# xmh1011/go-lsm

Hardware: AMD Instinct MI355X
Metric: GiB/s of device-resident .sst data-block bytes decoded to KV records (higher is better)
Workload: dtype u8; 1 GPU; decode 100000 x 4 KiB KV blocks per GPU (33 x 16 B key / 100 B value); grammar=KV (kv/kv.go:46-115), output=DESC (16 B record descriptors), blocks_per_gpu=100000, records_per_gpu=3300000, parsed_bytes_per_gpu=409200000, parallelism=dp1 (blocks round-robin, no collective)

## Files before the change

go-lsm_amd/csrc/decode.hip:

```cpp
#include <stdlib.h>
#include <string.h>

#include "common.h"

namespace lsm {
namespace {

constexpr uint32_t kChunk = 1024;
constexpr uint32_t kRingChunks = 8;
constexpr int kBlockLoadAux = 2;
constexpr uint32_t kBigLaunch = 400000;
template <uint32_t NCH, bool ARENA, bool BIG = false>
struct RingPolicy {
    static constexpr int load_aux = ((ARENA || BIG) && NCH == 8) ? 0 : kBlockLoadAux;
    static constexpr bool nt_desc = NCH == 8;
};
constexpr uint32_t kFitPad = 4096;
constexpr uint32_t kFitMin = 3072;

template <uint32_t NCH, bool ARENA>
__device__ __forceinline__ void store_desc(u32x4 *p, const u32x4 &d) {
    if (RingPolicy<NCH, ARENA>::nt_desc)
        __builtin_nontemporal_store(d, p);
    else
// ... 203 lines not shown
    constexpr uint32_t U = 1;
#pragma unroll 1
    for (uint32_t w0 = 0; w0 < nd; w0 += U * kWave) {
        uint32_t W[U], sb[U], kk[U], rr[U];
        int qv[U];
#pragma unroll
        for (uint32_t u = 0; u < U; u++) {
            const int q = (int)(4 * (w0 + u * kWave + lane)) - (int)lead;
            const uint32_t qc = q < 0 ? 0u : (uint32_t)q;
            const uint32_t r = rec(qc), o = qc - mul24(r, L);
            qv[u] = q;
            rr[u] = r;
            kk[u] = L - o;
            sb[u] = src0 + mul24(r, S) + o;
            W[u] = rb.word(sb[u] >> 2);
        }
        bool unal = false, cross = false;
#pragma unroll
        for (uint32_t u = 0; u < U; u++) {
            unal |= (sb[u] & 3) != 0;
            cross |= kk[u] < 4;
        }
        if (__ballot(unal)) {
#pragma unroll
            for (uint32_t u = 0; u < U; u++) W[u] = funnel(W[u], rb.word((sb[u] >> 2) + 1), sb[u]);
        }
        if (L < 4) {
#pragma unroll
            for (uint32_t u = 0; u < U; u++) {
                const uint32_t qc = qv[u] < 0 ? 0u : (uint32_t)qv[u];
                uint32_t x = 0;
                for (uint32_t t = 0; t < 4; t++) {
                    const uint32_t qq = qc + t;
                    if (qq < T) {
                        const uint32_t r = rec(qq);
                        x |= rb.u8(src0 + mul24(r, S) + (qq - mul24(r, L))) << (8 * t);
                    }
                }
                W[u] = x;
            }
        } else if (__ballot(cross)) {
#pragma unroll
            for (uint32_t u = 0; u < U; u++) {
                const uint32_t B = rb.u32(src0 + mul24(rr[u] + 1, S)), k = kk[u];
                W[u] = k < 4 ? (W[u] & ((1u << (8 * k)) - 1)) | (B << (8 * k)) : W[u];
            }
        }
#pragma unroll
        for (uint32_t u = 0; u < U; u++) {
            const uint32_t w = w0 + u * kWave + lane;
            const int q = qv[u];
            if (q >= 0 && (uint32_t)q + 4 <= T) {
                __builtin_nontemporal_store(W[u], &a0[w]);
            } else if (w < nd) {
                const uint32_t sh = q < 0 ? (uint32_t)(-q) : 0u;
                uint8_t *b = reinterpret_cast<uint8_t *>(a0 + w);
                for (uint32_t t = sh; t < 4 && (uint32_t)(q + (int)t) < T; t++)
                    b[t] = (uint8_t)(W[u] >> (8 * (t - sh)));
            }
        }
    }
}

template <uint32_t NCH, bool LIN>
__device__ __forceinline__ uint32_t arena_emit_batch(const RingBytes<NCH, LIN> &rb, uint32_t *tab,
                                                     uint8_t *out, uint32_t cnt, uint32_t src,
                                                     uint32_t len, uint64_t *out_off,
                                                     uint64_t cur) {
    const uint32_t lane = lane_id();
    const uint32_t l = lane < cnt ? len : 0u;
    uint32_t T;
    const uint32_t start = wave_excl_scan(l, &T);
    if (out_off && lane < cnt) out_off[lane] = cur + start;
    if (T == 0) return 0;
    uint32_t *tstart = tab, *tsrc = tab + 65;
    if (lane < cnt) {
        tstart[lane] = start;
        tsrc[lane] = src;
    }
    if (lane == 0) tstart[cnt] = T;
    __builtin_amdgcn_fence(__ATOMIC_RELEASE, "wavefront");
    __builtin_amdgcn_wave_barrier();
    __builtin_amdgcn_fence(__ATOMIC_ACQUIRE, "wavefront");
    const uint32_t lead = (uint32_t)((uintptr_t)out & 15);
    uint8_t *a0 = out - lead;
    const uint32_t nch = (lead + T + 15) >> 4;
#pragma unroll 1
    for (uint32_t c = lane; c < nch; c += kWave) {
        const int q0 = (int)(16 * c) - (int)lead;
        const uint32_t qf = q0 < 0 ? 0u : (uint32_t)q0;
        uint32_t lo = 0, hi = cnt;
        while (hi - lo > 1) {
            const uint32_t mid = (lo + hi) >> 1;
            if (tstart[mid] <= qf) lo = mid;
            else hi = mid;
        }
        uint32_t r = lo, rs0 = tstart[r], rs1 = tstart[r + 1], rsrc = tsrc[r];
        auto in_ring = [&]() { return rsrc >= rb.res_lo && rsrc + (rs1 - rs0) <= rb.res_hi; };
        auto seek = [&](uint32_t q) {
            while (rs1 <= q) {
                r++;
                rs0 = rs1;
                rs1 = tstart[r + 1];
                rsrc = tsrc[r];
            }
        };
        auto byte_at = [&](uint32_t q) -> uint32_t {
            seek(q);
            const uint32_t sb = rsrc + (q - rs0);
            return in_ring() ? rb.u8(sb) : rb.g8(sb);
        };
        u32x4 v{0, 0, 0, 0};
        if (q0 >= 0 && q0 + 16 <= (int)T && (uint32_t)q0 + 16 <= rs1) {
            const uint32_t sb = rsrc + ((uint32_t)q0 - rs0);
            if (in_ring())
                v = rb.u128(sb);
            else
                v = u32x4{rb.g32(sb), rb.g32(sb + 4), rb.g32(sb + 8), rb.g32(sb + 12)};
        } else {
#pragma unroll 1
            for (int t = 0; t < 16; t++) {
                const int q = q0 + t;
                if (q >= 0 && q < (int)T) {
                    const uint32_t b = byte_at((uint32_t)q) << (8 * (t & 3));
                    set_dword(v, (uint32_t)t >> 2, (t < 4 ? v.x : t < 8 ? v.y : t < 12 ? v.z : v.w) | b);
                }
            }
        }
        store_chunk(a0 + 16 * c, v, -q0, (int)T - q0);
    }
    __builtin_amdgcn_fence(__ATOMIC_RELEASE, "wavefront");
    __builtin_amdgcn_wave_barrier();
    __builtin_amdgcn_fence(__ATOMIC_ACQUIRE, "wavefront");
    return T;
}

typedef __attribute__((address_space(3))) uint32_t lds_u32_t;

template <uint32_t NCH, bool LIN>
__device__ __forceinline__ uint32_t arena_emit_batch_call(lds_u32_t *ring, rsrc_t rs, uint32_t res_lo,
                                                       uint32_t res_hi, lds_u32_t *tab,
                                                       uint8_t *out, uint32_t cnt, uint32_t src,
                                                       uint32_t len, uint64_t *out_off,
                                                       uint64_t cur) {
    RingBytes<NCH, LIN> rb{(const uint32_t *)ring, rs, res_lo, res_hi};
    return arena_emit_batch(rb, (uint32_t *)tab, out, cnt, src, len, out_off, cur);
}

struct ArenaCur {
    uint64_t k, v;
};

struct ChaseResume {
    uint32_t pos = 0, nr = 0, kprev = 0xFFFFFFFFu;
};
template <int G, uint32_t NCH, bool LIN, bool ARENA = false, bool BIG = false, bool PRE = false>
__device__ void decode_range_v2(const DecodeArgs &a, uint32_t *ring, uint64_t off, uint32_t n,
                                uint64_t base, uint32_t ncap, uint32_t &nr_out, int32_t &st_out,
                                uint32_t stop, uint32_t &pos_out, ArenaCur ac = {},
                                uint32_t *tab = nullptr, bool lin_rt = LIN,
                                const ChaseResume rs0 = {}) {
    static_assert(!PRE || (LIN && !ARENA), "a pre-landed ring is a DESC block that fits it");
    const bool lin = ARENA ? lin_rt : LIN;
    const uint32_t lane = lane_id();
    BlockReaderT<NCH, RingPolicy<NCH, ARENA, BIG>::load_aux> rd;
    rd.init(ring, a.in, off, n);
    RingBytes<NCH, LIN> rb{ring, rd.rsrc, 0, 0};

    auto word = [&](uint32_t w) -> uint32_t { return rb.word(w); };
    auto fld = [&](uint32_t p) -> uint32_t {
        return uni(rb.u32(rd.h + p));
    };
    auto lds_u32 = [&](uint32_t p) -> uint32_t {
        return rb.u32(rd.h + p);
    };

    uint32_t s_pos = 0, s_k = 0, s_v = 0, s_xlo = 0, s_xhi = 0, ns = 0, s_first = 0;
    uint32_t pos = rs0.pos, nr = rs0.nr, kprev = rs0.kprev, miss = 0, skip = 0;
    uint32_t pend = 0, pend_pos = 0, pend_k = 0, pend_v = 0;
    auto emit_run_arena = [&](uint32_t p0, uint32_t K, uint32_t V, uint32_t S, uint32_t cnt,
                              uint64_t slot0) {
#pragma unroll 1
        for (uint32_t f = G == LSM_GRAMMAR_V ? 1u : 0u; f < (G == LSM_GRAMMAR_IDX ? 1u : 2u);
             f++) {
            uint8_t *ar = f ? a.val_arena : a.key_arena;
            if (!ar) continue;
            uint64_t *ao = f ? a.val_arena_off : a.key_arena_off;
            const uint64_t cur = f ? ac.v : ac.k;
            const uint32_t L = f ? V : K;
            arena_emit_run(rb, ar + cur, rd.h + p0 + (f == 0 ? 4u : G == LSM_GRAMMAR_KV ? 8 + K : 4u),
                           S, L, cnt);
            if (ao)
                for (uint32_t i = lane; i < cnt; i += kWave) ao[slot0 + i] = cur + (uint64_t)i * L;
            if (f) ac.v += (uint64_t)cnt * L;
            else ac.k += (uint64_t)cnt * L;
        }
    };
    auto flush = [&]() {
        if (ns) {
            if (lane < ns) {
                const uint64_t ro = off + s_pos;
                u32x4 d;
                d.x = (uint32_t)ro;
                d.y = (uint32_t)(ro >> 32);
                d.z = s_k;
                d.w = s_v;
                store_desc<NCH, ARENA>(&a.desc[base + s_first + lane], d);
                if (G == LSM_GRAMMAR_IDX && a.idx_value)
                    a.idx_value[base + s_first + lane] = (int64_t)((uint64_t)s_xhi << 32 | s_xlo);
            }
            if (ARENA && ns > pend) {
                lds_u32_t *lring = (lds_u32_t *)ring, *ltab = (lds_u32_t *)tab;
#pragma unroll 1
                for (uint32_t f = G == LSM_GRAMMAR_V ? 1u : 0u;
                     f < (G == LSM_GRAMMAR_IDX ? 1u : 2u); f++) {
                    uint8_t *ar = f ? a.val_arena : a.key_arena;
                    if (!ar) continue;
                    uint64_t *ao = f ? a.val_arena_off : a.key_arena_off;
                    const uint64_t cur = f ? ac.v : ac.k;
                    const uint32_t src =
                        rd.h + s_pos + (f == 0 ? 4u : G == LSM_GRAMMAR_KV ? 8 + s_k : 4u);
                    const uint32_t t = arena_emit_batch_call<NCH, LIN>(
                        lring, rb.rs, rb.res_lo, rb.res_hi, ltab, ar + cur, ns - pend, src,
                        f ? s_v : s_k, ao ? ao + base + s_first : nullptr, cur);
                    if (f) ac.v += t;
                    else ac.k += t;
                }
            }
            ns = 0;
        }
    };
    uint32_t lim = PRE ? n : 0;
    auto need = [&](uint32_t p, uint32_t len) {
        if (PRE || (uint64_t)p + len <= lim) return;
        if (ARENA && !lin) {
            flush();
            if (pend) {
                emit_run_arena(pend_pos, pend_k, pend_v, 0, 1, base + nr - 1);
                pend = 0;
            }
        }
        rd.ensure(rd.h + p, lin ? rd.total : len);
        lim = rd.landed >= rd.nchunks ? n : rd.landed * kChunk - rd.h;
        if (ARENA) {
            rb.res_lo = (rd.hi_c > NCH ? rd.hi_c - NCH : 0u) * kChunk;
            rb.res_hi = rd.landed * kChunk;
        }
    };

    int32_t status = LSM_OK;
    for (;;) {
        const uint32_t rem = n - pos;
        if (rem == 0 || pos >= stop) break;
        if (rem < 4) {
            status = G == LSM_GRAMMAR_IDX ? LSM_ST_IDX_OVERRUN : LSM_ST_TRUNC_LEN_PREFIX;
            break;
        }
        need(pos, rem < kChunk ? rem : kChunk);
        uint32_t K = 0, V, S;
        uint64_t x = 0;
        if (G == LSM_GRAMMAR_V) {
            V = fld(pos);
            if (rem - 4 < V) { status = LSM_ST_TRUNC_VAL; break; }
            S = 4 + V;
        } else if (G == LSM_GRAMMAR_KV) {
            const bool sv = kprev <= kChunk - 8;
            K = fld(pos);
            const uint32_t vg = sv ? fld(pos + 4 + kprev) : 0u;
            if (K > kKeyCap) { status = LSM_ST_KEY_TOO_LONG; break; }
            if (rem - 4 < K) { status = LSM_ST_TRUNC_KEY; break; }
            const uint32_t vp = pos + 4 + K;
            const uint32_t rem2 = n - vp;
            if (rem2 < 4) { status = LSM_ST_TRUNC_VLEN; break; }
            if (sv && K == kprev) {
                V = vg;
            } else {
                need(vp, rem2 < kChunk ? rem2 : kChunk);
                V = fld(vp);
            }
            if (V > kValCap) { status = LSM_ST_VAL_TOO_LONG; break; }
            if (rem2 - 4 < V) { status = LSM_ST_TRUNC_VAL; break; }
            kprev = K;
            S = 8 + K + V;
        } else {
            K = fld(pos);
            if ((uint64_t)rem < 12ull + K) { status = LSM_ST_IDX_OVERRUN; break; }
            const uint32_t vp = pos + 4 + K;
            need(vp, 8);
            x = (uint64_t)fld(vp + 4) << 32 | fld(vp);
            V = 8;
            S = 12 + K;
        }
        if (nr >= ncap) { status = LSM_ST_CAPACITY; break; }
        if (ns == 0) s_first = nr;
        {
            const bool me = lane == ns;
            s_pos = me ? pos : s_pos;
            s_k = me ? K : s_k;
            s_v = me ? V : s_v;
            if (G == LSM_GRAMMAR_IDX) {
                s_xlo = me ? (uint32_t)x : s_xlo;
                s_xhi = me ? (uint32_t)(x >> 32) : s_xhi;
            }
        }
        if (++ns == kWave) flush();
        nr++;
        pos += S;

        if (skip) {
            skip--;
            if (G == LSM_GRAMMAR_KV && kprev <= kChunk - 8) {
                uint32_t vpos = to_vgpr(pos), kp = to_vgpr(kprev);
                while (nr < ncap) {
                    const uint32_t sb = rd.h + vpos, sv = sb + 4 + kp;
                    const uint32_t k = funnel(word(sb >> 2), word((sb >> 2) + 1), sb);
                    uint32_t v = funnel(word(sv >> 2), word((sv >> 2) + 1), sv);
                    if (!__ballot(k == kp) && __ballot(k <= kChunk - 8)) {
                        const uint32_t sw = sb + 4 + k;
                        v = funnel(word(sw >> 2), word((sw >> 2) + 1), sw);
// ... 94 lines not shown
        }
        if (ARENA && pend) {
            emit_run_arena(pend_pos, pend_k, pend_v, 0, 1, base + nr - 1);
            pend = 0;
        }
    }
    flush();
    nr_out = nr;
    st_out = status;
    pos_out = pos;
}

template <int G, uint32_t NCH, bool LIN, bool ARENA, bool BIG = false>
__device__ void decode_block_v2(const DecodeArgs &a, uint32_t b, uint32_t *ring, uint32_t *tab,
                                uint64_t off, uint32_t n, bool lin_rt = LIN) {
    uint64_t base, cap;
    record_slots<G>(a, b, off, n, base, cap);
    uint32_t nr, end;
    int32_t st;
    ArenaCur ac{};
    if (ARENA) {
        ac.k = a.arena_base ? uni64(a.arena_base[b]) : off;
        ac.v = ac.k;
    }
    decode_range_v2<G, NCH, LIN, ARENA, BIG>(a, ring, off, n, uni64(base),
                                        uni(cap < 0xFFFFFFFFull ? (uint32_t)cap : 0xFFFFFFFFu), nr,
                                        st, n, end, ac, tab, lin_rt);
    if (lane_id() == 0) {
        a.nrec[b] = nr;
        a.status[b] = st;
    }
}


template <int G, uint32_t NCH, bool BIG>
__device__ __forceinline__ void decode_block_lin(const DecodeArgs &a, uint32_t b, uint32_t *ring,
                                                 uint64_t off, uint32_t n) {
    static_assert(NCH * kChunk <= kKeyCap && NCH * kChunk <= kValCap, "caps hold for a block that fits");
    constexpr int AUX = RingPolicy<NCH, false, BIG>::load_aux;
    constexpr uint32_t R = MinRecord<G>::R;
    const uint32_t lane = lane_id();
    const uint32_t h = (uint32_t)off & 15;
    const uint32_t total = (h + n + 15) & ~15u;
    const uint32_t nchunks = (total + kChunk - 1) / kChunk;
    const rsrc_t rsrc = make_rsrc(a.in + (off - h), total);
    const uint32_t voff = lane * 16;
#pragma unroll
    for (uint32_t c = 0; c < NCH; c++)
        if (c < nchunks)
            __builtin_amdgcn_raw_ptr_buffer_load_lds(
                rsrc, (__attribute__((address_space(3))) void *)&ring[c * (kChunk / 4)], 16,
                voff + c * kChunk, 0, 0, AUX);
    uint64_t base64, cap64;
    record_slots<G>(a, b, off, n, base64, cap64);
    const uint64_t base = uni64(base64);
    const uint32_t ncap = uni(cap64 < 0xFFFFFFFFull ? (uint32_t)cap64 : 0xFFFFFFFFu);
    __asm__ __volatile__("s_waitcnt vmcnt(0)" ::: "memory");
    const RingBytes<NCH, true> rb{ring, rsrc, 0, 0};
    uint32_t pos = 0, nr = 0, K = 0, V = 8;
    if (n >= R) {
        bool ok0;
        if (G == LSM_GRAMMAR_V) {
            V = uni(rb.u32(h));
            ok0 = V <= n - 4;
        } else if (G == LSM_GRAMMAR_KV) {
            K = uni(rb.u32(h));
            ok0 = K <= n - 8;
            if (ok0) {
                V = uni(rb.u32(h + 4 + K));
                ok0 = V <= n - 8 - K;
            }
        } else {
            K = uni(rb.u32(h));
            ok0 = K <= n - 12;
        }
        if (ok0) {
            const uint32_t S = G == LSM_GRAMMAR_V ? 4 + V : G == LSM_GRAMMAR_KV ? 8 + K + V : 12 + K;
            const uint32_t p = lane * S;
            bool ok = p + S <= n && lane < ncap;
            uint64_t xx = 0;
            if (ok) {
                if (G == LSM_GRAMMAR_V) {
                    ok = rb.u32(h + p) == V;
                } else if (G == LSM_GRAMMAR_KV) {
                    ok = (int)(rb.u32(h + p) == K) & (int)(rb.u32(h + p + 4 + K) == V);
                } else {
                    ok = rb.u32(h + p) == K;
                    xx = (uint64_t)rb.u32(h + p + 8 + K) << 32 | rb.u32(h + p + 4 + K);
                }
            }
            const uint64_t m = __ballot(ok);
            const uint32_t j = m == ~0ull ? 64u : (uint32_t)__builtin_ctzll(~m);
            if (lane < j) {
                const uint64_t ro = off + p;
                u32x4 d;
                d.x = (uint32_t)ro;
                d.y = (uint32_t)(ro >> 32);
                d.z = K;
                d.w = V;
                store_desc<NCH, false>(&a.desc[base + lane], d);
                if (G == LSM_GRAMMAR_IDX && a.idx_value) a.idx_value[base + lane] = (int64_t)xx;
            }
            nr = j;
            pos = j * S;
        }
    }
    int32_t st = LSM_OK;
    if (pos != n) {
        uint32_t end;
        decode_range_v2<G, NCH, true, false, BIG, true>(
            a, ring, off, n, base, ncap, nr, st, n, end, {}, nullptr, true,
            ChaseResume{pos, nr, G == LSM_GRAMMAR_KV && nr ? K : 0xFFFFFFFFu});
    }
    if (lane == 0) {
        a.nrec[b] = nr;
        a.status[b] = st;
    }
}

template <int G, uint32_t NCH>
__device__ void decode_range_any(const DecodeArgs &a, uint32_t *ring, uint64_t off, uint32_t n,
                                 uint64_t base, uint32_t ncap, uint32_t &nr, int32_t &st,
                                 uint32_t stop = 0xFFFFFFFFu, uint32_t *end = nullptr) {
    uint32_t e;
    if (((off & 15) + (uint64_t)n + 15) / 16 * 16 <= NCH * kChunk)
        decode_range_v2<G, NCH, true>(a, ring, off, n, base, ncap, nr, st, stop, e);
    else
        decode_range_v2<G, NCH, false>(a, ring, off, n, base, ncap, nr, st, stop, e);
    if (end) *end = e;
}

template <int G, uint32_t NCH, bool ARENA, bool BIG = false, bool PAD = false>
__global__ __launch_bounds__(64) void decode_v2_kernel(DecodeArgs a) {
    static_assert(!PAD || (!ARENA && NCH == kRingChunks), "the pad is the 8 KiB DESC ring's");
    __shared__ __attribute__((aligned(16)))
    uint32_t ring[NCH * kChunk / 4 + 4 + (PAD ? kFitPad / 4 : 0)];
    __shared__ uint32_t tab[ARENA ? 129 : 1];
    const uint32_t b = a.order ? uni(a.order[blockIdx.x])
                               : NCH >= 16 ? xcd_linear(blockIdx.x, a.nblk) : blockIdx.x;
    const uint64_t off = uni64(a.blk_off[b]);
    const uint32_t n = uni(a.blk_len[b]);
    const bool lin = ((off & 15) + (uint64_t)n + 15) / 16 * 16 <= NCH * kChunk;
    if (ARENA) {
        decode_block_v2<G, NCH, false, true>(a, b, ring, tab, off, n, lin);
    } else if (lin && !BIG) {
        decode_block_lin<G, NCH, BIG>(a, b, ring, off, n);
    } else if (lin) {
        decode_block_v2<G, NCH, true, false, BIG>(a, b, ring, tab, off, n);
    } else {
        decode_block_v2<G, NCH, false, false, BIG>(a, b, ring, tab, off, n);
    }
}


constexpr uint32_t kScanThreads = 256;
constexpr uint32_t kScanPer = 2;
constexpr uint32_t kScanTile = kScanThreads * kScanPer;

__device__ __forceinline__ uint64_t plan_value(int mode, uint32_t len) {
    switch (mode) {
    case 0: return len / 4;
    case 1: return len / 8;
    case 2: return len / 12;
    default: return len;
    }
}

__device__ uint64_t block_excl_scan(uint64_t v, uint64_t *total) {
    __shared__ uint64_t wsum[kScanThreads / kWave];
    uint64_t wt;
    uint64_t x = wave_excl_scan64(v, &wt);
    uint32_t w = threadIdx.x / kWave;
    if (lane_id() == 0) wsum[w] = wt;
    __syncthreads();
    uint64_t pre = 0, tot = 0;
    for (uint32_t i = 0; i < kScanThreads / kWave; i++) {
        if (i < w) pre += wsum[i];
        tot += wsum[i];
    }
    __syncthreads();
    *total = tot;
    return x + pre;
}

__global__ __launch_bounds__(kScanThreads) void plan_tile_sums(int mode, const uint32_t *len,
                                                               uint32_t n, uint64_t *partial) {
    uint64_t s = 0;
    uint64_t i0 = (uint64_t)blockIdx.x * kScanTile + threadIdx.x * kScanPer;
    for (uint32_t j = 0; j < kScanPer; j++)
        if (i0 + j < n) s += plan_value(mode, len[i0 + j]);
    uint64_t tot;
    block_excl_scan(s, &tot);
    if (threadIdx.x == 0) partial[blockIdx.x] = tot;
}

constexpr uint32_t kPartThreads = 1024;

__global__ __launch_bounds__(kPartThreads) void plan_scan_partials(uint64_t *partial,
                                                                   uint32_t ntiles, uint64_t *out,
                                                                   uint32_t n) {
    __shared__ uint64_t wsum[kPartThreads / kWave];
    const uint32_t per = (ntiles + kPartThreads - 1) / kPartThreads, b = threadIdx.x * per;
    const uint32_t e = b + per < ntiles ? b + per : ntiles;
    uint64_t s = 0;
    for (uint32_t i0 = b; i0 < e; i0 += 8) {
        uint64_t v[8];
#pragma unroll
        for (uint32_t k = 0; k < 8; k++) v[k] = i0 + k < e ? partial[i0 + k] : 0;
#pragma unroll
        for (uint32_t k = 0; k < 8; k++) s += v[k];
    }
    uint64_t wt;
    const uint64_t wx = wave_excl_scan64(s, &wt);
    const uint32_t w = threadIdx.x / kWave;
    if (lane_id() == 0) wsum[w] = wt;
    __syncthreads();
    uint64_t pre = wx, tot = 0;
    for (uint32_t i = 0; i < kPartThreads / kWave; i++) {
        pre += i < w ? wsum[i] : 0;
        tot += wsum[i];
    }
    for (uint32_t i0 = b; i0 < e; i0 += 8) {
        uint64_t v[8];
#pragma unroll
        for (uint32_t k = 0; k < 8; k++) v[k] = i0 + k < e ? partial[i0 + k] : 0;
#pragma unroll
        for (uint32_t k = 0; k < 8; k++) {
            if (i0 + k < e) partial[i0 + k] = pre;
            pre += v[k];
        }
    }
    if (threadIdx.x == 0) out[n] = tot;
}

__global__ __launch_bounds__(kScanThreads) void plan_tile_apply(int mode, const uint32_t *len,
                                                                uint32_t n,
                                                                const uint64_t *partial,
                                                                uint64_t *out) {
    uint64_t vals[kScanPer];
    uint64_t s = 0;
    uint64_t i0 = (uint64_t)blockIdx.x * kScanTile + threadIdx.x * kScanPer;
    for (uint32_t j = 0; j < kScanPer; j++) {
        vals[j] = (i0 + j < n) ? plan_value(mode, len[i0 + j]) : 0;
        s += vals[j];
    }
    uint64_t tot;
    uint64_t pre = block_excl_scan(s, &tot) + partial[blockIdx.x];
    for (uint32_t j = 0; j < kScanPer; j++) {
        if (i0 + j < n) out[i0 + j] = pre;
        pre += vals[j];
    }
}

int plan_scan(int mode, const uint32_t *d_len, uint32_t n, uint64_t *d_out, void *ws,
              size_t ws_bytes, hipStream_t s) {
    uint32_t ntiles = (n + kScanTile - 1) / kScanTile;
    if (ntiles == 0) ntiles = 1;
    if (ws_bytes < (size_t)ntiles * 8 || (!ws && n)) return LSM_ESPACE;
    uint64_t *partial = static_cast<uint64_t *>(ws);
    if (n == 0) {
        LSM_HIP_CHECK(hipMemsetAsync(d_out, 0, 8, s));
        return 0;
    }
    hipLaunchKernelGGL(plan_tile_sums, dim3(ntiles), dim3(kScanThreads), 0, s, mode, d_len, n,
                       partial);
    hipLaunchKernelGGL(plan_scan_partials, dim3(1), dim3(kPartThreads), 0, s, partial, ntiles,
                       d_out, n);
    hipLaunchKernelGGL(plan_tile_apply, dim3(ntiles), dim3(kScanThreads), 0, s, mode, d_len, n,
                       partial, d_out);
    LSM_HIP_CHECK(hipGetLastError());
    return 0;
}

template <int G, bool ARENA, uint32_t NCH = kRingChunks>
int launch_decode(const DecodeArgs &a, hipStream_t s, bool fit = false) {
    static_assert(NCH >= 2, "a record header may straddle two ring chunks");
    constexpr bool kCanPad = !ARENA && NCH == kRingChunks && G != LSM_GRAMMAR_IDX;
    const bool big = !ARENA && NCH == kRingChunks && a.nblk > kBigLaunch && !a.order;
    if (kCanPad && fit && !big)
        hipLaunchKernelGGL((decode_v2_kernel<G, NCH, false, false, kCanPad>), dim3(a.nblk), dim3(kWave), 0, s, a);
    else if (big)
        hipLaunchKernelGGL((decode_v2_kernel<G, NCH, false, true>), dim3(a.nblk), dim3(kWave), 0, s, a);
    else
        hipLaunchKernelGGL((decode_v2_kernel<G, NCH, ARENA>), dim3(a.nblk), dim3(kWave), 0, s, a);
    LSM_HIP_CHECK(hipGetLastError());
    return 0;
}

constexpr uint32_t kSchedSub = 2;
constexpr uint32_t kSchedClasses = (33 - kSchedSub) << kSchedSub;
constexpr uint32_t kSchedThreads = 1024;
constexpr uint32_t kSchedPer = 16;
constexpr uint32_t kSchedTile = kSchedThreads * kSchedPer;
static_assert(kSchedClasses <= kSchedThreads, "one thread per class");

__device__ __forceinline__ uint32_t size_class(uint32_t n) {
    if (n < (1u << kSchedSub)) return n;
    const uint32_t l = 31 - __clz(n);
    return ((l - kSchedSub + 1) << kSchedSub) | ((n >> (l - kSchedSub)) & ((1u << kSchedSub) - 1));
}

constexpr uint32_t kSchedLaneWords = kSchedClasses * kWave;

__device__ __forceinline__ void sched_count(const uint32_t *len, uint32_t nblk, uint32_t t0,
                                            uint32_t (*h2)[kWave], uint32_t n[kSchedPer]) {
    for (uint32_t i = threadIdx.x; i < kSchedLaneWords; i += kSchedThreads) (&h2[0][0])[i] = 0;
// ... 940 lines not shown
}
size_t scan_workspace_bytes(uint32_t n) {
    const size_t ntiles = (n + kScanTile - 1) / kScanTile;
    return (ntiles ? ntiles : 1) * 8;
}
}

extern "C" uint64_t lsm_max_records(int grammar, uint64_t len) {
    switch (grammar) {
    case LSM_GRAMMAR_V: return len / 4;
    case LSM_GRAMMAR_KV: return len / 8;
    case LSM_GRAMMAR_IDX: return len / 12;
    default: return 0;
    }
}

extern "C" size_t lsm_plan_workspace_bytes(uint32_t nblk) {
    size_t ntiles = (nblk + kScanTile - 1) / kScanTile;
    return (ntiles ? ntiles : 1) * 8;
}

extern "C" int lsm_plan_rec_base(lsm_ctx *ctx, int grammar, const uint32_t *d_blk_len,
                                 uint32_t nblk, uint64_t *d_rec_base, void *d_workspace,
                                 size_t ws_bytes, void *stream) {
    if (!ctx || !d_rec_base || (nblk && !d_blk_len)) return LSM_EINVAL;
    if (grammar < LSM_GRAMMAR_V || grammar > LSM_GRAMMAR_IDX) return LSM_EINVAL;
    int mode = grammar == LSM_GRAMMAR_V ? 0 : grammar == LSM_GRAMMAR_KV ? 1 : 2;
    return plan_scan(mode, d_blk_len, nblk, d_rec_base, d_workspace, ws_bytes,
                     static_cast<hipStream_t>(stream));
}

extern "C" int lsm_plan_arena_base(lsm_ctx *ctx, const uint32_t *d_blk_len, uint32_t nblk,
                                   uint64_t *d_arena_base, void *d_workspace, size_t ws_bytes,
                                   void *stream) {
    if (!ctx || !d_arena_base || (nblk && !d_blk_len)) return LSM_EINVAL;
    return plan_scan(3, d_blk_len, nblk, d_arena_base, d_workspace, ws_bytes,
                     static_cast<hipStream_t>(stream));
}

__global__ __launch_bounds__(256) void compact_kernel(int grammar, const uint64_t *blk_off,
                                                      uint32_t nblk, const u32x4 *desc,
                                                      const int64_t *idx, const uint64_t *rec_base,
                                                      const uint32_t *nrec, const uint64_t *out_base,
                                                      u32x4 *dense, int64_t *dense_idx) {
    const uint32_t b = uni(blockIdx.x * 4 + threadIdx.x / kWave);
    if (b >= nblk) return;
    const uint32_t R = grammar == LSM_GRAMMAR_V ? 4 : grammar == LSM_GRAMMAR_KV ? 8 : 12;
    const uint64_t src = rec_base ? uni64(rec_base[b]) : uni64(blk_off[b]) / R;
    const uint64_t dst = uni64(out_base[b]);
    const uint32_t n = uni(nrec[b]);
    for (uint32_t i = lane_id(); i < n; i += kWave) {
        dense[dst + i] = __builtin_nontemporal_load(&desc[src + i]);
        if (dense_idx) dense_idx[dst + i] = idx[src + i];
    }
}

extern "C" int lsm_compact_records(lsm_ctx *ctx, int grammar, const uint64_t *d_blk_off,
                                   uint32_t nblk, const lsm_decode_out *out, lsm_rec_desc *d_dense,
                                   int64_t *d_dense_idx, uint64_t *d_dense_base, void *d_workspace,
                                   size_t ws_bytes, void *stream) {
    if (!ctx || !out || !d_dense_base) return LSM_EINVAL;
    if (grammar < LSM_GRAMMAR_V || grammar > LSM_GRAMMAR_IDX) return LSM_EINVAL;
    if (nblk && (!out->desc || !out->nrec || !d_dense || (!out->rec_base && !d_blk_off)))
        return LSM_EINVAL;
    if (d_dense_idx && (grammar != LSM_GRAMMAR_IDX || !out->idx_value)) return LSM_EINVAL;
    hipStream_t s = static_cast<hipStream_t>(stream);
    const int rc = plan_scan(3, out->nrec, nblk, d_dense_base, d_workspace, ws_bytes, s);
    if (rc) return rc;
    if (nblk == 0) return 0;
    hipLaunchKernelGGL(compact_kernel, dim3((nblk + 3) / 4), dim3(256), 0, s, grammar, d_blk_off,
                       nblk, reinterpret_cast<const u32x4 *>(out->desc), out->idx_value,
                       out->rec_base, out->nrec, d_dense_base, reinterpret_cast<u32x4 *>(d_dense),
                       d_dense_idx);
    LSM_HIP_CHECK(hipGetLastError());
    return 0;
}

static int decode_blocks_8k(lsm_ctx *ctx, int grammar, const uint8_t *d_in,
                            const uint64_t *d_blk_off, const uint32_t *d_blk_len, uint32_t nblk,
                            const lsm_decode_out *out, void *stream, bool fit) {
    if (!ctx || !out) return LSM_EINVAL;
    if (nblk == 0) return 0;
    if (!d_in || !d_blk_off || !d_blk_len || !out->desc || !out->nrec || !out->status)
        return LSM_EINVAL;
    if (grammar < LSM_GRAMMAR_V || grammar > LSM_GRAMMAR_IDX) return LSM_EINVAL;
    bool arena = out->key_arena || out->val_arena;
    DecodeArgs a;
    a.in = d_in;
    a.blk_off = d_blk_off;
    a.blk_len = d_blk_len;
    a.nblk = nblk;
    a.desc = reinterpret_cast<u32x4 *>(out->desc);
    a.rec_base = out->rec_base;
    a.nrec = out->nrec;
    a.status = out->status;
    a.idx_value = out->idx_value;
    a.key_arena = out->key_arena;
    a.val_arena = out->val_arena;
    a.arena_base = out->arena_base;
    a.key_arena_off = out->key_arena_off;
    a.val_arena_off = out->val_arena_off;
    a.order = nullptr;
    hipStream_t s = static_cast<hipStream_t>(stream);
    switch (grammar) {
    case LSM_GRAMMAR_V: return arena ? launch_decode<LSM_GRAMMAR_V, true>(a, s)
                                     : launch_decode<LSM_GRAMMAR_V, false>(a, s, fit);
    case LSM_GRAMMAR_KV: return arena ? launch_decode<LSM_GRAMMAR_KV, true>(a, s)
                                      : launch_decode<LSM_GRAMMAR_KV, false>(a, s, fit);
    default: return arena ? launch_decode<LSM_GRAMMAR_IDX, true>(a, s)
                          : launch_decode<LSM_GRAMMAR_IDX, false>(a, s);
    }
}

extern "C" int lsm_decode_blocks(lsm_ctx *ctx, int grammar, const uint8_t *d_in,
                                 const uint64_t *d_blk_off, const uint32_t *d_blk_len,
                                 uint32_t nblk, const lsm_decode_out *out, void *stream) {
    return decode_blocks_8k(ctx, grammar, d_in, d_blk_off, d_blk_len, nblk, out, stream, false);
}

extern "C" int lsm_decode_blocks_hinted(lsm_ctx *ctx, int grammar, const uint8_t *d_in,
                                        const uint64_t *d_blk_off, const uint32_t *d_blk_len,
                                        uint32_t nblk, uint32_t max_blk_len,
                                        const lsm_decode_out *out, void *stream) {
    if (max_blk_len <= 32 * 1024)
        return decode_blocks_8k(ctx, grammar, d_in, d_blk_off, d_blk_len, nblk, out, stream,
                                max_blk_len > kFitMin &&
                                    max_blk_len + 15 <= kRingChunks * kChunk);
    if (!ctx || !out) return LSM_EINVAL;
    if (nblk == 0) return 0;
    if (!d_in || !d_blk_off || !d_blk_len || !out->desc || !out->nrec || !out->status)
        return LSM_EINVAL;
    if (grammar < LSM_GRAMMAR_V || grammar > LSM_GRAMMAR_IDX) return LSM_EINVAL;
    const bool arena = out->key_arena || out->val_arena;
    DecodeArgs a;
    a.in = d_in;
    a.blk_off = d_blk_off;
    a.blk_len = d_blk_len;
    a.nblk = nblk;
    a.desc = reinterpret_cast<u32x4 *>(out->desc);
    a.rec_base = out->rec_base;
    a.nrec = out->nrec;
    a.status = out->status;
    a.idx_value = out->idx_value;
    a.key_arena = out->key_arena;
    a.val_arena = out->val_arena;
    a.arena_base = out->arena_base;
    a.key_arena_off = out->key_arena_off;
    a.val_arena_off = out->val_arena_off;
    a.order = nullptr;
    hipStream_t s = static_cast<hipStream_t>(stream);
    constexpr uint32_t R = 2 * kRingChunks;
    switch (grammar) {
    case LSM_GRAMMAR_V: return arena ? launch_decode<LSM_GRAMMAR_V, true, R>(a, s)
                                     : launch_decode<LSM_GRAMMAR_V, false, R>(a, s);
    case LSM_GRAMMAR_KV: return arena ? launch_decode<LSM_GRAMMAR_KV, true, R>(a, s)
                                      : launch_decode<LSM_GRAMMAR_KV, false, R>(a, s);
    default: return arena ? launch_decode<LSM_GRAMMAR_IDX, true, R>(a, s)
                          : launch_decode<LSM_GRAMMAR_IDX, false, R>(a, s);
    }
}

extern "C" size_t lsm_decode_schedule_workspace_bytes(uint32_t nblk) {
    const uint64_t ntile = ((uint64_t)nblk + kSchedTile - 1) / kSchedTile;
    return 4ull * kSchedClasses * ntile + 4ull * nblk + 16;
}

extern "C" int lsm_decode_blocks_scheduled(lsm_ctx *ctx, int grammar, const uint8_t *d_in,
                                           const uint64_t *d_blk_off, const uint32_t *d_blk_len,
                                           uint32_t nblk, const lsm_decode_out *out,
                                           void *d_workspace, size_t ws_bytes, void *stream) {
    if (!ctx || !out) return LSM_EINVAL;
    if (nblk == 0) return 0;
    if (!d_in || !d_blk_off || !d_blk_len || !out->desc || !out->nrec || !out->status)
        return LSM_EINVAL;
    if (grammar < LSM_GRAMMAR_V || grammar > LSM_GRAMMAR_IDX) return LSM_EINVAL;
    if (!d_workspace || ws_bytes < lsm_decode_schedule_workspace_bytes(nblk)) return LSM_ESPACE;
    hipStream_t s = static_cast<hipStream_t>(stream);
    const uint32_t ntile = (nblk + kSchedTile - 1) / kSchedTile;
    uint32_t *order = static_cast<uint32_t *>(d_workspace);
    uint32_t *hist = order + nblk;
    hipLaunchKernelGGL(sched_hist_kernel, dim3(ntile), dim3(kSchedThreads), 0, s, d_blk_len, nblk,
                       hist);
    hipLaunchKernelGGL(sched_scatter_kernel, dim3(ntile), dim3(kSchedThreads), 0, s, d_blk_len, nblk,
                       ntile, hist, order);
    LSM_HIP_CHECK(hipGetLastError());
    const bool arena = out->key_arena || out->val_arena;
    DecodeArgs a;
    a.in = d_in;
    a.blk_off = d_blk_off;
    a.blk_len = d_blk_len;
    a.nblk = nblk;
    a.desc = reinterpret_cast<u32x4 *>(out->desc);
    a.rec_base = out->rec_base;
    a.nrec = out->nrec;
    a.status = out->status;
    a.idx_value = out->idx_value;
    a.key_arena = out->key_arena;
    a.val_arena = out->val_arena;
    a.arena_base = out->arena_base;
    a.key_arena_off = out->key_arena_off;
    a.val_arena_off = out->val_arena_off;
    a.order = order;
    constexpr uint32_t R = kRingChunks / 4;
    switch (grammar) {
    case LSM_GRAMMAR_V: return arena ? launch_decode<LSM_GRAMMAR_V, true, R>(a, s)
                                     : launch_decode<LSM_GRAMMAR_V, false, R>(a, s);
    case LSM_GRAMMAR_KV: return arena ? launch_decode<LSM_GRAMMAR_KV, true, R>(a, s)
                                      : launch_decode<LSM_GRAMMAR_KV, false, R>(a, s);
    default: return arena ? launch_decode<LSM_GRAMMAR_IDX, true, R>(a, s)
                          : launch_decode<LSM_GRAMMAR_IDX, false, R>(a, s);
    }
}


extern "C" size_t lsm_wal_replay_workspace_bytes(uint32_t nwal, uint32_t max_wal_len) {
    const uint64_t segs = max_wal_len ? ((uint64_t)max_wal_len + kWalSeg - 1) / kWalSeg : 1;
    const uint64_t n = (uint64_t)nwal * segs;
    return (size_t)(n * (2 * sizeof(WalSeg) + 8 + 2ull * kWalSegSlots * 16) + 64);
}

extern "C" int lsm_wal_replay(lsm_ctx *ctx, const uint8_t *d_wal, const uint64_t *d_wal_off,
                              const uint32_t *d_wal_len, uint32_t nwal, uint32_t max_wal_len,
                              const lsm_decode_out *out, void *d_workspace, size_t ws_bytes,
                              void *stream) {
    if (!ctx || !out) return LSM_EINVAL;
    if (nwal == 0) return 0;
    if (!d_wal || !d_wal_off || !d_wal_len || !out->desc || !out->nrec || !out->status ||
        !d_workspace || out->key_arena || out->val_arena || nwal > 65535)
        return LSM_EINVAL;
    if (ws_bytes < lsm_wal_replay_workspace_bytes(nwal, max_wal_len)) return LSM_ESPACE;
    WalArgs a;
    a.wal = d_wal;
    a.wal_off = d_wal_off;
    a.wal_len = d_wal_len;
    a.nwal = nwal;
    a.max_len = max_wal_len;
    a.segs = max_wal_len ? (max_wal_len + kWalSeg - 1) / kWalSeg : 1;
    a.out = *out;
    const uint64_t n = (uint64_t)nwal * a.segs;
    uint8_t *ws = static_cast<uint8_t *>(d_workspace);
    a.scratch = reinterpret_cast<u32x4 *>(ws);
    a.seg = reinterpret_cast<WalSeg *>(ws + n * 2 * kWalSegSlots * 16);
    a.fin = reinterpret_cast<uint32_t *>(ws + n * 2 * (kWalSegSlots * 16 + sizeof(WalSeg)));
    hipStream_t s = static_cast<hipStream_t>(stream);
    hipLaunchKernelGGL(wal_seg_lanes_kernel, dim3(a.segs, nwal), dim3(kWave), 0, s, a);
    hipLaunchKernelGGL(wal_stitch_kernel, dim3(nwal), dim3(kWave), 0, s, a);
    hipLaunchKernelGGL(wal_compact_kernel, dim3(a.segs, nwal), dim3(256), 0, s, a);
    LSM_HIP_CHECK(hipGetLastError());
    return 0;
}

extern "C" size_t lsm_decode_sst_workspace_bytes(uint32_t nfile) {
    return (size_t)nfile * (sizeof(SstWork) + 12) + 16;
}

extern "C" int lsm_decode_sst(lsm_ctx *ctx, const uint8_t *d_img, const uint64_t *d_file_off,
                              const uint64_t *d_file_len, uint32_t nfile,
                              const uint64_t *d_rec_base, lsm_sst_meta *d_meta,
                              lsm_rec_desc *d_idx_desc, int64_t *d_idx_value,
                              lsm_rec_desc *d_data_desc, void *d_workspace, size_t ws_bytes,
                              void *stream) {
    if (!ctx) return LSM_EINVAL;
    if (nfile == 0) return 0;
    if (nfile > 65535 || !d_img || !d_file_off || !d_file_len || !d_meta || !d_idx_desc ||
        !d_idx_value || !d_data_desc || !d_workspace)
        return LSM_EINVAL;
    if (ws_bytes < lsm_decode_sst_workspace_bytes(nfile)) return LSM_ESPACE;
    hipStream_t s = static_cast<hipStream_t>(stream);
    SstArgs a;
    a.img = d_img;
    a.file_off = d_file_off;
    a.file_len = d_file_len;
    a.nfile = nfile;
    a.rec_base = d_rec_base;
    a.meta = d_meta;
    a.idx_desc = reinterpret_cast<u32x4 *>(d_idx_desc);
    a.idx_value = d_idx_value;
    a.data_desc = reinterpret_cast<u32x4 *>(d_data_desc);
    a.work = static_cast<SstWork *>(d_workspace);
    a.fail = reinterpret_cast<uint32_t *>(static_cast<uint8_t *>(d_workspace) +
                                          (size_t)nfile * sizeof(SstWork));
    LSM_HIP_CHECK(hipMemsetAsync(a.fail, 0xFF, (size_t)nfile * 12, s));
    constexpr uint32_t kSstWgs = 16384;
    uint32_t g = (kSstWgs + nfile - 1) / nfile;
    if (g > 64) g = 64;
    if (g == 0) g = 1;
    hipLaunchKernelGGL(sst_index_kernel, dim3(g, nfile), dim3(256), 0, s, a);
    hipLaunchKernelGGL(sst_tail_kernel, dim3(nfile), dim3(256), 0, s, a);
    LSM_HIP_CHECK(hipGetLastError());
    return 0;
}
```

Baseline: 5197 GiB/s.

## Add multi-wave split decode kernel that verifies uniform-stride records in parallel

Adds a four-wave decode kernel for the V and KV grammars. Each wave loads its own ring window and checks whether the block is a run of identically sized records, in which case all waves write descriptors directly. Otherwise wave 0 falls back to the serial chase, reusing chunks already landed in the ring. Blocks that fit the ring (4 KiB blocks here) still go to the one-wave linear path, so the workload mainly sees a launch with four times as many threads per block and idle extra waves.

```diff
diff --git a/go-lsm_amd/csrc/decode.hip b/go-lsm_amd/csrc/decode.hip
--- a/go-lsm_amd/csrc/decode.hip
+++ b/go-lsm_amd/csrc/decode.hip
@@ -379,7 +379,7 @@
 };
 
 struct ChaseResume {
-    uint32_t pos = 0, nr = 0, kprev = 0xFFFFFFFFu;
+    uint32_t pos = 0, nr = 0, kprev = 0xFFFFFFFFu, landed = 0;
 };
 template <int G, uint32_t NCH, bool LIN, bool ARENA = false, bool BIG = false, bool PRE = false>
 __device__ void decode_range_v2(const DecodeArgs &a, uint32_t *ring, uint64_t off, uint32_t n,
@@ -392,6 +392,7 @@
     const uint32_t lane = lane_id();
     BlockReaderT<NCH, RingPolicy<NCH, ARENA, BIG>::load_aux> rd;
     rd.init(ring, a.in, off, n);
+    if (!PRE) rd.hi_c = rd.landed = rs0.landed < rd.nchunks ? rs0.landed : rd.nchunks;
     RingBytes<NCH, LIN> rb{ring, rd.rsrc, 0, 0};
 
     auto word = [&](uint32_t w) -> uint32_t { return rb.word(w); };
@@ -792,6 +793,165 @@
     }
 }
 
+constexpr uint32_t kSplitWaves = 4;
+
+template <int G, uint32_t W>
+__global__ __launch_bounds__(W * kWave) void decode_split_kernel(DecodeArgs a) {
+    constexpr uint32_t NCH = 2 * kRingChunks;
+    constexpr uint32_t SEGC = NCH / W;
+    constexpr uint32_t WB = SEGC * kChunk;
+    static_assert(G != LSM_GRAMMAR_IDX, "IDX keeps the one-wave kernel");
+    static_assert(W * SEGC == NCH && W <= 16, "the first round's windows are the ring's chunks");
+    __shared__ __attribute__((aligned(16))) uint32_t ring[NCH * kChunk / 4 + 4];
+    __shared__ uint32_t tab[1];
+    __shared__ uint32_t s_bad, s_over[W];
+    const uint32_t lane = lane_id(), wave = uni(threadIdx.x / kWave);
+    if (threadIdx.x == 0) __atomic_store_n(&s_bad, 0u, __ATOMIC_RELAXED);
+    __syncthreads();
+    const uint32_t b = xcd_linear(blockIdx.x, a.nblk);
+    const uint64_t off = uni64(a.blk_off[b]);
+    const uint32_t n = uni(a.blk_len[b]);
+    const uint32_t h = (uint32_t)off & 15;
+    const uint64_t tot = ((uint64_t)h + n + 15) & ~(uint64_t)15;
+    if (tot <= NCH * kChunk) {
+        if (wave == 0) decode_block_lin<G, NCH, false>(a, b, ring, off, n);
+        return;
+    }
+    const uint32_t total = (uint32_t)(tot > 0xFFFFFFF0ull ? 0xFFFFFFF0ull : tot);
+    const rsrc_t brs = make_rsrc(a.in + (off - h), total);
+    uint32_t *wr = ring + wave * (WB / 4);
+    const uint32_t voff = lane * 16;
+#pragma unroll
+    for (uint32_t c = 0; c < SEGC; c++)
+        __builtin_amdgcn_raw_ptr_buffer_load_lds(
+            brs, (__attribute__((address_space(3))) void *)&wr[c * (kChunk / 4)], 16,
+            voff + wave * WB + c * kChunk, 0, 0, kBlockLoadAux);
+    uint64_t base = 0;
+    uint32_t ncap = 0, K = 0, V = 0, S = 0, m = 0;
+    bool split = false;
+    {
+        const uint32_t w0 = ld_b32(brs, lane * 4);
+        auto head = [&](uint32_t p) -> uint32_t {
+            const uint32_t i = p >> 2;
+            return funnel((uint32_t)__builtin_amdgcn_readlane((int)w0, (int)i),
+                          (uint32_t)__builtin_amdgcn_readlane((int)w0, (int)i + 1), p);
+        };
+        bool ok0;
+        if (G == LSM_GRAMMAR_V) {
+            V = head(h);
+            ok0 = V <= n - 4;
+            S = 4 + V;
+        } else {
+            K = head(h);
+            ok0 = K <= kKeyCap && K <= n - 8;
+            if (ok0) {
+                const uint32_t p = h + 4 + K;
+                V = p <= 248 ? head(p)
+                             : uni(funnel(ld_b32(brs, p & ~3u), ld_b32(brs, (p & ~3u) + 4), p));
+                ok0 = V <= kValCap && V <= n - 8 - K;
+            }
+            S = 8 + K + V;
+        }
+        if (ok0 && S <= NCH * kChunk - 32 && n <= 0x7FFFFFFFu) {
+            uint64_t base64, cap64;
+            record_slots<G>(a, b, off, n, base64, cap64);
+            base = uni64(base64);
+            ncap = uni(cap64 < 0xFFFFFFFFull ? (uint32_t)cap64 : 0xFFFFFFFFu);
+            m = n / S;
+            split = m <= ncap;
+        }
+    }
+    __asm__ __volatile__("s_waitcnt vmcnt(0)" ::: "memory");
+    bool over = false;
+    if (split) {
+        const RingBytes<SEGC, true> rb{wr, brs, 0, 0};
+        const uint32_t nwin = (total + WB - 1) / WB;
+        bool bad = false;
+        for (uint32_t g = wave; g < nwin; g += W) {
+            const uint32_t wlo = g * WB, whi = wlo + WB < total ? wlo + WB : total;
+            const uint32_t jlo = wlo <= h ? 0u : (wlo - h + S - 1) / S;
+            uint32_t jhi = (whi - h + S - 1) / S;
+            jhi = jhi < m ? jhi : m;
+            if (jlo >= jhi) continue;
+            if (g != wave) {
+                if (uni(__atomic_load_n(&s_bad, __ATOMIC_RELAXED))) break;
+                over = true;
+#pragma unroll
+                for (uint32_t c = 0; c < SEGC; c++)
+                    __builtin_amdgcn_raw_ptr_buffer_load_lds(
+                        brs, (__attribute__((address_space(3))) void *)&wr[c * (kChunk / 4)], 16,
+                        voff + wlo + c * kChunk, 0, 0, kBlockLoadAux);
+                __asm__ __volatile__("s_waitcnt vmcnt(0)" ::: "memory");
+            }
+            auto word = [&](uint32_t x) -> uint32_t {
+                const bool in = x + 4 <= wlo + WB;
+                uint32_t v = rb.u32(in ? x - wlo : 0u);
+                if (!in) v = funnel(ld_b32(brs, x & ~3u), ld_b32(brs, (x & ~3u) + 4), x);
+                return v;
+            };
+            bool ok = true;
+            for (uint32_t j = jlo + lane; j < jhi; j += kWave) {
+                const uint32_t x = h + j * S;
+                if (G == LSM_GRAMMAR_V)
+                    ok &= word(x) == V;
+                else
+                    ok &= (int)(word(x) == K) & (int)(word(x + 4 + K) == V);
+            }
+            bad = __ballot(!ok) != 0;
+            if (bad) break;
+        }
+        if (bad && lane == 0) __atomic_store_n(&s_bad, 1u, __ATOMIC_RELAXED);
+    }
+    if (lane == 0) s_over[wave] = over;
+    __syncthreads();
+    if (split && uni(__atomic_load_n(&s_bad, __ATOMIC_RELAXED)) == 0) {
+        for (uint32_t i = threadIdx.x; i < m; i += W * kWave) {
+            const uint64_t ro = off + (uint64_t)i * S;
+            u32x4 d;
+            d.x = (uint32_t)ro;
+            d.y = (uint32_t)(ro >> 32);
+            d.z = K;
+            d.w = V;
+            store_desc<NCH, false>(&a.desc[base + i], d);
+        }
+        if (wave != 0) return;
+        uint32_t nr = 0, end;
+        int32_t st = LSM_OK;
+        const uint32_t rem = n - m * S;
+        if (rem)
+            decode_range_v2<G, NCH, true>(a, ring, off + (uint64_t)m * S, rem, base + m, ncap - m,
+                                          nr, st, rem, end);
+        if (lane == 0) {
+            a.nrec[b] = m + nr;
+            a.status[b] = st;
+        }
+        return;
+    }
+    if (wave != 0) return;
+    ChaseResume rs;
+    for (rs.landed = 0; rs.landed < NCH; rs.landed += SEGC)
+        if (uni(s_over[rs.landed / SEGC])) break;
+    uint64_t base64, cap64;
+    record_slots<G>(a, b, off, n, base64, cap64);
+    uint32_t nr, end;
+    int32_t st;
+    decode_range_v2<G, NCH, false>(a, ring, off, n, uni64(base64),
+                                   uni(cap64 < 0xFFFFFFFFull ? (uint32_t)cap64 : 0xFFFFFFFFu), nr,
+                                   st, n, end, {}, tab, false, rs);
+    if (lane == 0) {
+        a.nrec[b] = nr;
+        a.status[b] = st;
+    }
+}
+
+template <int G>
+int launch_decode_split(const DecodeArgs &a, hipStream_t s) {
+    hipLaunchKernelGGL((decode_split_kernel<G, kSplitWaves>), dim3(a.nblk),
+                       dim3(kSplitWaves * kWave), 0, s, a);
+    LSM_HIP_CHECK(hipGetLastError());
+    return 0;
+}
+
 
 constexpr uint32_t kScanThreads = 256;
 constexpr uint32_t kScanPer = 2;
@@ -2038,9 +2198,9 @@
     constexpr uint32_t R = 2 * kRingChunks;
     switch (grammar) {
     case LSM_GRAMMAR_V: return arena ? launch_decode<LSM_GRAMMAR_V, true, R>(a, s)
-                                     : launch_decode<LSM_GRAMMAR_V, false, R>(a, s);
+                                     : launch_decode_split<LSM_GRAMMAR_V>(a, s);
     case LSM_GRAMMAR_KV: return arena ? launch_decode<LSM_GRAMMAR_KV, true, R>(a, s)
-                                      : launch_decode<LSM_GRAMMAR_KV, false, R>(a, s);
+                                      : launch_decode_split<LSM_GRAMMAR_KV>(a, s);
     default: return arena ? launch_decode<LSM_GRAMMAR_IDX, true, R>(a, s)
                           : launch_decode<LSM_GRAMMAR_IDX, false, R>(a, s);
     }
```

Result: no change. 5150 GiB/s (-0.9%).
